# gt1/daccord

Measured on AMD Instinct MI355X. Metric: corrected Mbase/s (whole node), synthetic 20x PacBio piles, higher is better.
Workload: dtype u64+f64; 1 GPU; BASELINE.json configs[1] (10k A-reads x 10 kb x 20x, k=14, one MI355X): synthetic 10000 A-reads x 10000 b x 20x, 15% error (ins 80/del 13.3/sub 6.7), k=14, w=40, a=10, tspace=100; piles_total=10000, piles_rank0=10000, overlaps_rank0=319252, windows_rank0=9969965, trace_blocks_rank0=17906701, corrected_bases_total=90715992

## Files before the change

daccord_amd/csrc/capi.hip:

```cpp
#include <hip/hip_runtime.h>
#include <vector>
#include <string>
#include <cstring>
#include <cstdio>
#include <cstdlib>
#include <new>
#include "../../include/daccord_hip.h"
#include "batch_plan.hpp"
#include "host_tables.hpp"
#include "window_kernels.hpp"
#include "trace_kernel.hpp"
#include "vote_kernel.hpp"
#include "emit_record.hpp"
#include "context.hpp"

using namespace dacc;


struct PrepBatch
{
	DevOvl const * ovl; uint64_t novl; uint8_t const * trace; uint32_t trace_bytes;
	uint32_t * blk_ovl; uint32_t * blk_b0;
};

// ... 297 lines not shown

int dacc_create(dacc_ctx ** out, dacc_params const * p)
{
	if ( !out || !p ) return DACC_EINVAL;
	*out = 0;
	if ( p->klow < 3 || p->khigh > 16 || p->klow > p->khigh || !p->w || !p->a || p->w > DACC_WMAX || p->minfilterfreq < 0 ||
	     p->maxfilterfreq < p->minfilterfreq || p->tspace <= 0 || p->tspace > 512 )
		return DACC_EINVAL;
	if ( readTierSwitches().conflict() ) return DACC_EINVAL;
	int ndev = 0;
	if ( hipGetDeviceCount(&ndev) != hipSuccess || ndev <= 0 || p->device < 0 || p->device >= ndev )
		return DACC_ENODEV;
	if ( hipSetDevice(p->device) != hipSuccess ) return DACC_ENODEV;
	dacc_ctx * c = new (std::nothrow) dacc_ctx;
	if ( !c ) return DACC_ENOMEM;
	c->par = *p; c->device = p->device;
	c->sw = readTierSwitches();
	char const * sc = getenv("DACC_SCHED"); c->env_sched = sc ? atoi(sc) : 1;
	{ char const * td = getenv("DACC_TRACE_DYN"); c->env_trdyn = !(td && td[0] == '0'); }
	char const * ta = getenv("DACC_T7_ADAPT"); c->env_t7adapt = !(ta && ta[0] == '0');
	char const * dr = getenv("DACC_DEBUG_RETRY"); c->env_dbgretry = (dr && dr[0] == '1');
	{ char const * fn = getenv("DACC_FEAS_NEED"); c->env_feasneed = (fn && fn[0] == '0') ? 0u : 1u; }
	{ char const * tf = getenv("DACC_TIE_FAST"); c->env_tiefast = (tf && tf[0] == '0') ? 0u : 1u; }
	if ( hipStreamCreate(&c->stream.h) != hipSuccess ) { delete c; return DACC_EHIP; }
	{ int lo = 0, hi = 0; hipDeviceGetStreamPriorityRange(&lo,&hi); if ( hipStreamCreateWithPriority(&c->stream2.h,hipStreamNonBlocking,hi) != hipSuccess ) { delete c; return DACC_EHIP; } }
	hipEventCreateWithFlags(&c->evFirstTier.h,hipEventDisableTiming); hipEventCreateWithFlags(&c->evEarlyGeneric.h,hipEventDisableTiming); hipEventCreateWithFlags(&c->evPrescan.h,hipEventDisableTiming);
	for ( Event & e : c->ev ) hipEventCreate(&e.h);
	for ( Event & e : c->evEmit ) hipEventCreate(&e.h);
	for ( Event & e : c->evLong ) hipEventCreate(&e.h);
	for ( Event & e : c->evslot ) hipEventCreate(&e.h);
	for ( dacc_ctx::Stage & S : c->st ) hipEventCreate(&S.done.h);
	hipEventCreate(&c->h2dend.h);
	*out = c;
	return DACC_OK;
}

void dacc_destroy(dacc_ctx * c)
{
	if ( !c ) return;
	hipSetDevice(c->device);
	hipStreamSynchronize(c->stream); hipStreamSynchronize(c->stream2);
	delete c;
}

char const * dacc_last_error(dacc_ctx * c) { return c ? c->err.c_str() : "null context"; }

// ... 72 lines not shown
static dacc_ctx::Stage * ranOf(dacc_ctx * c, TierId const id) { return c->st[id].ran ? &c->st[id] : static_cast<dacc_ctx::Stage *>(0); }

struct Pass
{
	WindowBatch WB;
	uint32_t const * list = 0;
	int lastslot = -1;
	bool early = false;
	uint32_t herr[4] = {0,0,0,0};
	size_t symbytes = 0;
};

static WindowBatch windowBatch(dacc_ctx * c)
{
	BatchPlan & BP = c->BP; WindowBatch WB;
	WB.P = c->P; WB.T = c->T; WB.C = BP.caps; WB.bps = c->d_bps.p; WB.boff = c->d_boff.p; WB.rlen = c->d_rlen.p;
	WB.piles = c->d_piles.p; WB.npiles = BP.piles.size(); WB.ovl = c->d_ovl.p; WB.wt_b = c->d_wt_b.p; WB.wt_e = c->d_wt_e.p;
	WB.nwindows = BP.nwindows; WB.wrec = c->d_wrec.p; WB.wout = c->d_wout.p; WB.arena = c->d_arena.p; WB.prof = c->d_prof.p;
	return WB;
}
static FastBatch stageBatch(dacc_ctx * c, WindowBatch const & WB, uint32_t const id, bool const chain = true)
{
	FastBatch FB; FB.W = WB; FB.F = c->BP.stageCaps(id); FB.dpsq_vst = c->d_vst.p; FB.tab32 = c->d_tab32.p; FB.feasneed = c->env_feasneed; FB.tiefast = c->env_tiefast;
	if ( !chain ) return FB;
	FB.hand = c->handcap ? c->d_hand.p : static_cast<uint64_t *>(0); FB.handctr = c->d_handctr.p; FB.handcap = c->handcap; FB.handwords = c->TP.handwords;
#if defined(DACC_LEDGER)
	{ char const * lm = getenv("DACC_LEDGER_MASK"); FB.ledger = lm ? static_cast<uint32_t>(strtoul(lm,0,0)) : 0u; }
#endif
	return FB;
}
static void handsOn(FastBatch & FB, uint32_t * const handon, uint8_t * const slab) { FB.retry = handon; FB.gslab = slab; FB.gstride = FB.F.gbytes; }

static void growHandOver(dacc_ctx * c)
{
	if ( !(c->nruns && c->handwant > c->handcap && !c->nohand) ) return;
	uint64_t cap = c->handwant;
	{ size_t fr = 0, tot = 0; if ( hipMemGetInfo(&fr,&tot) == hipSuccess ) { uint64_t const lim = (static_cast<uint64_t>(fr)/2) / (static_cast<uint64_t>(c->TP.handwords)*8ull); if ( cap > lim ) cap = lim; } else (void)hipGetLastError(); }
	while ( cap && c->d_hand.ensure(static_cast<size_t>(cap)*c->TP.handwords) != hipSuccess ) { (void)hipGetLastError(); cap = cap > 65536 ? cap/2 : 0; }
	c->handcap = static_cast<uint32_t>(cap); c->handwant = cap;
}

static int enqueuePrepAndTrace(dacc_ctx * c)
{
	BatchPlan & BP = c->BP; hipStream_t const s = c->stream;
	HIPCHK(hipMemsetAsync(c->d_err.p,0,4*sizeof(uint32_t),s));
	HIPCHK(hipEventRecord(c->ev[0],s));
// ... 682 lines not shown
```

daccord_amd/csrc/context.hpp:

```cpp
#ifndef DACC_CONTEXT_HPP
#define DACC_CONTEXT_HPP
#include <hip/hip_runtime.h>
#include <cstdlib>
#include <string>
#include <vector>
#include "../../include/daccord_hip.h"
#include "batch_plan.hpp"
#include "host_tables.hpp"
#include "window_main.hpp"
#include "vote_kernel.hpp"

namespace dacc {

template<typename T>
struct DevBuf
{
	T * p = 0; size_t cap = 0;
	DevBuf() = default; DevBuf(DevBuf const &) = delete; DevBuf & operator=(DevBuf const &) = delete;
	~DevBuf() { release(); }
	hipError_t ensure(size_t n)
	{
		if ( n <= cap ) return hipSuccess;
		if ( p ) { hipFree(p); p = 0; cap = 0; }
		hipError_t const e = hipMalloc(reinterpret_cast<void **>(&p),n*sizeof(T));
// ... 53 lines not shown
	std::vector<uint32_t> h_rlen;
	BatchPlan BP;
	DevBuf<DevPile> d_piles; DevBuf<DevOvl> d_ovl; DevBuf<uint32_t> d_ovl_pile; DevBuf<uint8_t> d_trace;
	DevBuf<uint32_t> d_blk_ovl, d_blk_b0, d_wt_b, d_wt_e;
	DevBuf<uint8_t> d_wrec; DevBuf<WindowOut> d_wout; DevBuf<uint8_t> d_arena;
	DevBuf<uint8_t> d_has, d_oc, d_outsym, d_pilebad; DevBuf<uint16_t> d_ld0; DevBuf<uint32_t> d_ocs, d_nfrag, d_err;
	DevBuf<VoteFragment> d_frags; DevBuf<uint64_t> d_fragbase; DevBuf<uint64_t> d_prof;
	DevBuf<uint64_t> d_vst; DevBuf<uint32_t> d_tab32; DevBuf<uint8_t> d_gslab, d_arena2; DevBuf<uint64_t> d_trslab;
	DevBuf<uint32_t> d_retry[TIER_NSLOTS], d_work, d_gearly, d_pregen, d_pregen2, d_pregenlist, d_small;
	DevBuf<uint8_t> d_longslab;
	DevBuf<uint32_t> d_longhand[2];
	DevBuf<uint64_t> d_hand; DevBuf<uint32_t> d_handctr; uint32_t handcap = 0; uint64_t handwant = 0, nruns = 0; bool nohand = false, oom = false;
	bool noslab = false;
	bool tier7_adapt_off = false;
	TierSwitches sw = {}; TierPipeline TP = {};
	struct Stage { bool ran = false; uint32_t grid = 0; DevBuf<uint32_t> handon; DevBuf<uint8_t> slab; Event done; uint32_t const * in = 0;  } st[TIER_NROWS];
	uint32_t nlong[2] = {0,0};
	bool longran[2] = {false,false}; Event evLong[4];
	uint32_t retry_grid = 0, early_grid = 0; int sched = 0;
	uint32_t tr_grid = 0, tr_lds = 0, tr_words = 0, tr_lanes = 0, trace_bytes = 0, win_grid = 0;
	int env_sched = 1, env_dbgretry = 0, env_t7adapt = 1, env_trdyn = 1;
	uint32_t env_feasneed = 1;
	uint32_t env_tiefast = 1;
	std::vector<uint32_t> retry_flags;
	std::vector<dacc_fragment> frags; std::string bases;
	std::vector<int32_t> pile_status; std::vector<std::string> pile_errors; std::string pile_errors_joined;
	std::vector<uint32_t> h_nfrag; std::vector<VoteFragment> h_frags; HostBuf<uint8_t> h_outsym;
	dacc_timing timing = {};
};

}

struct dacc_ctx : dacc::Context {};
#endif
```

daccord_amd/csrc/fast_diag.hpp:

```cpp
#ifndef DACC_FAST_DIAG_HPP
#define DACC_FAST_DIAG_HPP
#if defined(DACC_EMUL)
#include <cstdint>
#include <cstdio>
#include <cstdlib>
#include <vector>
#include <algorithm>
#endif

namespace dacc {

#if defined(DACC_EMUL)
struct FastStats { enum { N = 33 }; uint32_t v[N]; void clear() { for ( int i = 0; i < N; ++i ) v[i] = 0; } void mx(int i, uint32_t x) { if ( x > v[i] ) v[i] = x; } void add(int i, uint32_t x) { v[i] += x; } };
static FastStats g_fstats;
static inline void fstats_dump(int const tier)
{
	static FILE * sf = 0; static bool tried = false;
	if ( !tried ) { tried = true; char const * fn = getenv("DACC_EMUL_STATS"); if ( fn ) sf = fopen(fn,"w"); }
	if ( sf ) { fprintf(sf,"%d",tier); for ( int i = 0; i < FastStats::N; ++i ) fprintf(sf," %u",g_fstats.v[i]); fprintf(sf,"\n"); fflush(sf); }
}
static inline FILE * ftrav_file() { static FILE * f = 0; static bool tried = false; if ( !tried ) { tried = true; char const * fn = getenv("DACC_EMUL_TRAV"); if ( fn ) f = fopen(fn,"w"); } return f; }
#define FSTAT_MX(i,x) g_fstats.mx(i,x)
#define FSTAT_ADD(i,x) g_fstats.add(i,x)
struct FeasIters { std::vector<uint32_t> it, ln; void clear() { it.clear(); ln.clear(); } };
static FeasIters g_feasit;
static inline void feasit_dump()
{
	static FILE * f = 0; static bool tried = false;
	if ( !tried ) { tried = true; char const * fn = getenv("DACC_EMUL_FEAS"); if ( fn ) f = fopen(fn,"w"); }
	if ( !f ) { g_feasit.clear(); return; }
	std::vector<uint32_t> const & it = g_feasit.it; std::vector<uint32_t> const & ln = g_feasit.ln;
	uint64_t tot = 0, lock = 0, locksorted = 0;
	for ( size_t i = 0; i < it.size(); ++i ) tot += it[i];
	for ( size_t i = 0; i < it.size(); i += 64 ) { uint32_t m = 0; for ( size_t q = i; q < it.size() && q < i+64; ++q ) m = std::max(m,it[q]); lock += m; }
	std::vector< std::pair<uint32_t,uint32_t> > P; for ( size_t i = 0; i < it.size(); ++i ) P.push_back(std::make_pair(ln[i],it[i]));
	std::stable_sort(P.begin(),P.end(),[](std::pair<uint32_t,uint32_t> const & a, std::pair<uint32_t,uint32_t> const & b){ return a.first > b.first; });
	for ( size_t i = 0; i < P.size(); i += 64 ) { uint32_t m = 0; for ( size_t q = i; q < P.size() && q < i+64; ++q ) m = std::max(m,P[q].second); locksorted += m; }
	uint64_t lockcls = 0;
	{
		std::vector< std::pair<uint32_t,uint32_t> > Q; for ( size_t i = 0; i < it.size(); ++i ) { uint32_t c = 0; while ( (2u<<c) <= ln[i] ) ++c; Q.push_back(std::make_pair(c,it[i])); }
		std::stable_sort(Q.begin(),Q.end(),[](std::pair<uint32_t,uint32_t> const & a, std::pair<uint32_t,uint32_t> const & b){ return a.first > b.first; });
		for ( size_t i = 0; i < Q.size(); i += 64 ) { uint32_t m = 0; for ( size_t q = i; q < Q.size() && q < i+64; ++q ) m = std::max(m,Q[q].second); lockcls += m; }
	}
	fprintf(f,"%zu %llu %llu %llu %llu\n",it.size(),(unsigned long long)tot,(unsigned long long)lock,(unsigned long long)locksorted,(unsigned long long)lockcls);
// ... 82 lines not shown
static FeasNeedAudit g_feasneed;
#define FEAS_NEED_UNIT(s,rev,lo0,hi0,lo1,hi1) { if ( !feascount ) g_feasneed.unit(s,rev,lo0,hi0,lo1,hi1); }
#define FEAS_NEED_PROBE(s,rev,p) g_feasneed.probe(s,rev,p);
#define FEAS_NEED_LINK(a,b) g_feasneed.link(a,b);
#define FEAS_OVER() { if ( !feascount ) over(128); }
#define FEAS_NEED_PASS() { if ( lane == 0 ) ++g_feasneed.passes; }
#define FEAS_NEED_DUMP() { if ( lane == 0 && !feascount && g_feasneed.on() ) { FeasNeedAudit & A_ = g_feasneed; ++A_.ntrav; A_.recF += nwF; A_.recR += nwR; A_.mids += nmid; A_.hlek += (H <= static_cast<int64_t>(k)); \
	for ( uint32_t c_ = 0; c_ < nF; ++c_ ) A_.insF += (L.fnode()[c_] != 0xFFFF && L.parF()[c_] != SNONE); for ( uint32_t c_ = 0; c_ < nL; ++c_ ) A_.insL += (L.lnode()[c_] != 0xFFFF && L.parL()[c_] != SNONE); A_.dump(); } }
#else
#define FEAS_ITERS(t,len,n)
#define FEAS_DUMP()
#define FEAS_UNITS(W,nu)
#define FEAS_NODE(j,len,pp,nrows,f)
#define FEAS_FAIL(j,len)
#define FEAS_CASES_DUMP()
#define FEAS_NEED_UNIT(s,rev,lo0,hi0,lo1,hi1)
#define FEAS_NEED_PROBE(s,rev,p)
#define FEAS_NEED_LINK(a,b)
#define FEAS_NEED_DUMP()
#define FEAS_NEED_PASS()
#define FEAS_OVER() over(128);
#define FSTAT_MX(i,x)
#define FSTAT_ADD(i,x)
#endif
}
#endif
```

daccord_amd/csrc/fast_tiers.hpp:

```cpp
#ifndef DACC_FAST_TIERS_HPP
#define DACC_FAST_TIERS_HPP
#include <cstdint>
#include "tier_pipeline.hpp"

namespace dacc {

template<int TIER> struct FastTier;
#if !defined(DACC_RCH01)
#define DACC_RCH01 2
#endif
template<> struct FastTier<1> { typedef uint8_t id_t; typedef uint8_t sid_t; enum : uint32_t { smax = 250, gw = 1, wcapg = 1024, rch = DACC_RCH01, fch = 4, fnw = 2, fnc = 40, idmax = 250, rpstcap = 256, lstr = 64, maxs = 32, precap = 1024, ncap = 776, scap = 112, lcap = 960, wcap = 1024, rccap = 144, fcap = 192, siqcap = 56, blcap = 96, seqcap = 32, psiq = 8, consrow = 64, lscrids = 2048, wide = 0, mins = 0, gmem = 0 }; };
template<> struct FastTier<0> { typedef uint8_t id_t; typedef uint8_t sid_t; enum : uint32_t { smax = 250, gw = 1, wcapg = 768, rch = DACC_RCH01, fch = 4, fnw = 2, fnc = 32, idmax = 250, rpstcap = 256, lstr = 64, maxs = 28, precap = 576, ncap = 524, scap = 88, lcap = 640, wcap = 768, rccap = 96, fcap = 128, siqcap = 56, blcap = 96, seqcap = 32, psiq = 8, consrow = 64, lscrids = 2048, wide = 0, mins = 0, gmem = 0 }; };
template<> struct FastTier<7> { typedef uint8_t id_t; typedef uint8_t sid_t; enum : uint32_t { smax = 250, gw = 1, wcapg = 896, rch = DACC_RCH01, fch = 4, fnw = 2, fnc = 32, idmax = 250, rpstcap = 256, lstr = 64, maxs = 28, precap = 704, ncap = 640, scap = 104, lcap = 800, wcap = 896, rccap = 112, fcap = 148, siqcap = 56, blcap = 96, seqcap = 32, psiq = 8, consrow = 64, lscrids = 2048, wide = 0, mins = 0, gmem = 0 }; };
#if !defined(DACC_T2_NCAP)
#define DACC_T2_NCAP 1536
#endif
#if !defined(DACC_T2_LCAP)
#define DACC_T2_LCAP 2032
#endif
template<> struct FastTier<2> { typedef uint8_t id_t; typedef uint8_t sid_t; enum : uint32_t { smax = 250, gw = 1, wcapg = 3072, rch = 4, fch = 4, fnw = 4, fnc = 64, idmax = 250, rpstcap = 256, lstr = 64, maxs = 96, precap = 2048, ncap = DACC_T2_NCAP, scap = 232, lcap = DACC_T2_LCAP, wcap = 3072, rccap = 256, fcap = 192, siqcap = 96, blcap = 96, seqcap = 48, psiq = 10, consrow = 96, lscrids = 2560, wide = 0, mins = 0, gmem = 0 }; };
template<> struct FastTier<6> { typedef uint8_t id_t; typedef uint8_t sid_t; enum : uint32_t { smax = 250, gw = 1, wcapg = 2048, rch = 2, fch = 8, fnw = 3, fnc = 40, idmax = 250, rpstcap = 256, lstr = 128, maxs = 40, precap = 1024, ncap = 1024, scap = 248, lcap = 1280, wcap = 2048, rccap = 256, fcap = 256, siqcap = 96, blcap = 96, seqcap = 48, psiq = 10, consrow = 96, lscrids = 2560, wide = 0, mins = 0, gmem = 0 }; };

template<> struct FastTier<3> { typedef uint16_t id_t; typedef uint16_t sid_t; enum : uint32_t { smax = 1000, gw = 1, wcapg = 8192, rch = 8, fch = 16, fnw = 4, fnc = 72, idmax = 4000, rpstcap = 768, lstr = 128, maxs = 96, precap = 4096, ncap = 2048, scap = 1024, lcap = 4096, wcap = 8192, rccap = 2048, fcap = 512, siqcap = 256, blcap = 128, seqcap = 48, psiq = 10, consrow = 96, lscrids = 2560, wide = 0, mins = 0, gmem = 0 }; };

template<> struct FastTier<4> { typedef uint8_t id_t; typedef uint8_t sid_t; enum : uint32_t { smax = 250, gw = 1, wcapg = 608, rch = 4, fch = 4, fnw = 2, fnc = 40, idmax = 250, rpstcap = 256, lstr = 64, maxs = 96, precap = 2048, ncap = 256, scap = 48, lcap = 256, wcap = 608, rccap = 128, fcap = 96, siqcap = 56, blcap = 96, seqcap = 48, psiq = 10, consrow = 96, lscrids = 2560, wide = 0, mins = 0, gmem = 0 }; };

template<> struct FastTier<5> { typedef uint16_t id_t; typedef uint8_t sid_t; enum : uint32_t { smax = 250, gw = 0, wcapg = 0, rch = 8, fch = 16, fnw = 4, fnc = 72, idmax = 4000, rpstcap = 768, lstr = 128, maxs = 64, precap = 4096, ncap = 1792, scap = 250, lcap = 2048, wcap = 2040, rccap = 512, fcap = 512, siqcap = 256, blcap = 128, seqcap = 48, psiq = 10, consrow = 96, lscrids = 2560, wide = 0, mins = 0, gmem = 0 }; };

template<> struct FastTier<8> { typedef uint16_t id_t; typedef uint8_t sid_t; enum : uint32_t { smax = 250, gw = 1, wcapg = 6144, rch = 4, fch = 8, fnw = 4, fnc = 64, idmax = 4000, rpstcap = 768, lstr = 128, maxs = 40, precap = 3072, ncap = 2304, scap = 248, lcap = 3072, wcap = 6144, rccap = 640, fcap = 512, siqcap = 96, blcap = 128, seqcap = 96, psiq = 10, consrow = 128, lscrids = 2560, wide = 1, mins = 0, gmem = 0 }; };

template<> struct FastTier<9> { typedef uint16_t id_t; typedef uint16_t sid_t; enum : uint32_t { smax = 500, gw = 1, wcapg = 8192, rch = 16, fch = 16, fnw = 4, fnc = 72, idmax = 4000, rpstcap = 768, lstr = 128, maxs = 64, precap = 4096, ncap = 3072, scap = 512, lcap = 4096, wcap = 8192, rccap = 2048, fcap = 1024, siqcap = 256, blcap = 128, seqcap = 96, psiq = 10, consrow = 128, lscrids = 2560, wide = 1, mins = 0, gmem = 0 }; };

template<> struct FastTier<10> { typedef uint16_t id_t; typedef uint8_t sid_t; enum : uint32_t { smax = 250, gw = 1, wcapg = 6144, rch = 4, fch = 8, fnw = 4, fnc = 64, idmax = 4000, rpstcap = 768, lstr = 128, maxs = 64, precap = 2560, ncap = 2048, scap = 248, lcap = 3072, wcap = 6144, rccap = 896, fcap = 512, siqcap = 128, blcap = 128, seqcap = 48, psiq = 10, consrow = 96, lscrids = 2560, wide = 0, mins = 0, gmem = 0 }; };

template<> struct FastTier<11> { typedef uint16_t id_t; typedef uint8_t sid_t; enum : uint32_t { smax = 250, gw = 1, wcapg = 4096, rch = 4, fch = 8, fnw = 4, fnc = 72, idmax = 4000, rpstcap = 768, lstr = 128, maxs = 96, precap = 4096, ncap = 1536, scap = 248, lcap = 2048, wcap = 4096, rccap = 640, fcap = 384, siqcap = 128, blcap = 128, seqcap = 48, psiq = 10, consrow = 96, lscrids = 2560, wide = 0, mins = 0, gmem = 0 }; };

template<> struct FastTier<12> { typedef uint16_t id_t; typedef uint16_t sid_t; enum : uint32_t { smax = 1000, gw = 1, wcapg = 8192, rch = 8, fch = 16, fnw = 4, fnc = 72, idmax = 4000, rpstcap = 768, lstr = 128, maxs = 250, precap = 8192, ncap = 2048, scap = 1024, lcap = 4096, wcap = 8192, rccap = 2048, fcap = 512, siqcap = 256, blcap = 128, seqcap = 48, psiq = 10, consrow = 96, lscrids = 2560, wide = 0, mins = 96, gmem = 0 }; };

template<> struct FastTier<13> { typedef uint16_t id_t; typedef uint16_t sid_t; enum : uint32_t { smax = 2000, gw = 1, wcapg = 16384, rch = 16, fch = 16, fnw = 4, fnc = 72, idmax = 4000, rpstcap = 768, lstr = 128, maxs = 250, precap = 16384, ncap = 4096, scap = 2048, lcap = 8192, wcap = 16384, rccap = 4096, fcap = 1024, siqcap = 512, blcap = 128, seqcap = 48, psiq = 10, consrow = 96, lscrids = 4096, wide = 0, mins = 0, gmem = 1 }; };
template<> struct FastTier<14> { typedef uint16_t id_t; typedef uint16_t sid_t; enum : uint32_t { smax = 1000, gw = 1, wcapg = 16384, rch = 16, fch = 16, fnw = 4, fnc = 72, idmax = 4000, rpstcap = 768, lstr = 128, maxs = 250, precap = 16384, ncap = 6144, scap = 1024, lcap = 8192, wcap = 16384, rccap = 4096, fcap = 2048, siqcap = 512, blcap = 128, seqcap = 96, psiq = 10, consrow = 128, lscrids = 4096, wide = 1, mins = 0, gmem = 1 }; };
template<> struct FastTier<15> { typedef uint16_t id_t; typedef uint16_t sid_t; enum : uint32_t { smax = 2000, gw = 1, wcapg = 32768, rch = 16, fch = 16, fnw = 4, fnc = 72, idmax = 4000, rpstcap = 768, lstr = 128, maxs = 1000, precap = 16384, ncap = 4096, scap = 2048, lcap = 8192, wcap = 32768, rccap = 4096, fcap = 1024, siqcap = 512, blcap = 128, seqcap = 48, psiq = 10, consrow = 96, lscrids = 4096, wide = 0, mins = 250, gmem = 1 }; };

static_assert(uint32_t(FastTier<15>::mins) == VDEEP_MINS && uint32_t(FastTier<13>::maxs) == VDEEP_MINS,"the very deep stage takes what the last stage refuses at its string count");
template<> struct FastTier<16> { typedef uint16_t id_t; typedef uint16_t sid_t; enum : uint32_t { smax = 4000, gw = 1, wcapg = 65536, rch = 16, fch = 16, fnw = 4, fnc = 72, idmax = 8000, rpstcap = 768, lstr = 128, maxs = 2000, precap = 16384, ncap = 8190, scap = 4096, lcap = 16384, wcap = 65536, rccap = 4096, fcap = 1024, siqcap = 512, blcap = 128, seqcap = 48, psiq = 10, consrow = 96, lscrids = 4096, wide = 0, mins = 250, gmem = 1 }; };
static_assert(uint32_t(FastTier<16>::mins) == VDEEP_MINS && uint32_t(FastTier<15>::maxs) == XDEEP_MINS,"the deepest stage takes what the very deep stage hands on with more than 250 strings");
template<> struct FastTier<18> { typedef uint16_t id_t; typedef uint16_t sid_t; enum : uint32_t { smax = 12000, gw = 1, wcapg = 131072, rch = 16, fch = 16, fnw = 4, fnc = 72, idmax = 24000, rpstcap = 768, lstr = 128, maxs = 5001, precap = 16384, ncap = 16384, scap = 12288, lcap = 49152, wcap = 131072, rccap = 4096, fcap = 1024, siqcap = 512, blcap = 128, seqcap = 48, psiq = 10, consrow = 96, lscrids = 4096, wide = 0, mins = 250, gmem = 1 }; };
static_assert(uint32_t(FastTier<18>::mins) == VDEEP_MINS && uint32_t(FastTier<16>::maxs) == FDEEP_MINS,"the full-depth stage takes what the deepest stage hands on with more than 250 strings");
template<> struct FastTier<19> { typedef uint16_t id_t; typedef uint16_t sid_t; enum : uint32_t { smax = 4000, gw = 1, wcapg = 98304, rch = 64, fch = 16, fnw = 4, fnc = 72, idmax = 8000, rpstcap = 768, lstr = 128, maxs = 1000, precap = 16384, ncap = 8190, scap = 4096, lcap = 16384, wcap = 98304, rccap = 16384, fcap = 2048, siqcap = 512, blcap = 128, seqcap = 96, psiq = 10, consrow = 128, lscrids = 16384, wide = 1, mins = 250, gmem = 1 }; };
static_assert(uint32_t(FastTier<19>::mins) == VDEEP_MINS && uint32_t(FastTier<14>::maxs) == VDEEP_MINS && uint32_t(FastTier<19>::maxs) == FastTier<15>::maxs,"the wide deep stage takes what the last stage of a wide batch refuses at its string count");
template<> struct FastTier<17> { typedef uint16_t id_t; typedef uint16_t sid_t; enum : uint32_t { smax = 1000, gw = 1, wcapg = 16384, rch = 16, fch = 16, fnw = 8, fnc = 72, idmax = 4000, rpstcap = 768, lstr = 256, maxs = 250, precap = 16384, ncap = 6144, scap = 1024, lcap = 8192, wcap = 16384, rccap = 4096, fcap = 4096, siqcap = 512, blcap = 128, seqcap = 96, psiq = 10, consrow = 128, lscrids = 4096, wide = 1, mins = 0, gmem = 1, oneslab = 1 }; };
template<typename CT, typename = void> struct FastOneSlab { enum : uint32_t { value = 0 }; };
template<typename CT> struct FastOneSlab<CT,decltype(void(CT::oneslab))> { enum : uint32_t { value = (CT::oneslab != 0) ? 1u : 0u }; };

}
#endif
```

daccord_amd/csrc/fast_window.hpp:

```cpp
#ifndef DACC_FAST_WINDOW_HPP
#define DACC_FAST_WINDOW_HPP
#include "wave.hpp"
#include "dev_types.hpp"
#include "arena.hpp"
#include "window_main.hpp"
#include "tier_pipeline.hpp"
#include "fast_tiers.hpp"
#include "fast_layout.hpp"
#include "fast_diag.hpp"
#include "emit_record.hpp"

namespace dacc {

enum { WS_RETRY = 4 };
enum { FNOPAR = 0xFF };
enum { FSEQCAP = 48 };

struct FastBatch
{
	WindowBatch W;
	FastCaps F = {};
	uint64_t const * dpsq_vst = 0;
	uint32_t * retry = 0;
	uint32_t * gearly = 0;
// ... 31 lines not shown
struct FastEngine
{
	typedef typename CT::id_t id_t;
	typedef typename CT::sid_t sid_t;
	enum : uint32_t { SB = 8u*sizeof(sid_t), SMASK = (1u<<SB)-1u, SNONE = SMASK, SMAX = CT::smax };
	FastLds<CT> L; DevTables T; DevParams P;
	uint32_t nrows, nsup;
	uint64_t const * vst;
	enum : bool { GW = (CT::gw != 0) };
	uint8_t * gslab;
	uint32_t const * gtab;
	struct G4 { uint32_t x, y, z, w; };
	int lane; uint32_t flags;
#if defined(DACC_LEDGER)
	uint32_t ledger;
#endif
	uint64_t * prof;
	uint32_t mao, k; uint64_t kmask;
	uint32_t npre, nlast, nn, nmfirst, nmlast;
	uint32_t n0, npool, nlinks, nwF, nwR;
	uint32_t nF, nL;
	uint32_t feasneed;
	uint32_t tiefast;

#if defined(DACC_EMUL)
	bool feascount, feasapplied; uint32_t nwFall, nwRall;
	DEV bool feasNeedOn() const { char const * e = getenv("DACC_FEAS_NEED"); return !(e && e[0] == '0'); }
	DEV bool tieFastOn() const { char const * e = getenv("DACC_TIE_FAST"); return !(e && e[0] == '0'); }
#else
	static constexpr bool feascount = false;
	DEV bool feasNeedOn() const { return feasneed != 0; }
	DEV bool tieFastOn() const { return tiefast != 0; }
#endif
#if defined(DACC_EMUL)
	DEV void over_(uint32_t b, int line) { flags |= b; static char const * ov = getenv("DACC_EMUL_OVER"); if ( ov ) fprintf(stderr,"[over] tier maxs=%d line %d bits 0x%x nn=%u n0=%u npool=%u nF=%u nL=%u nwF=%u nwR=%u rstop=%u\n",int(CT::maxs)*10000+int(CT::ncap),line,b,nn,n0,npool,nF,nL,nwF,nwR,rstop); }
	#define over(b) over_(b,__LINE__)
#else
	DEV void over(uint32_t b) { flags |= b; }
#endif
#if defined(DACC_PROFILE) && !defined(DACC_EMUL)
	DEV void pcount(int id, uint64_t v) { if ( prof ) atomicAdd(reinterpret_cast<unsigned long long *>(prof+id),static_cast<unsigned long long>(v)); }
	DEV uint64_t pclock() { return clock64(); }
#else
	DEV void pcount(int, uint64_t) {}
	DEV uint64_t pclock() { return 0; }
#endif

#if defined(DACC_PROFILE) && !defined(DACC_EMUL)
	#define SITE_T0 uint64_t _ps = clock64();
	#define SITE_RESET { _ps = clock64(); }
	#define SITE(id) { uint64_t const _n = clock64(); if ( prof && lane == static_cast<int>(__builtin_ctzll(__builtin_amdgcn_ballot_w64(true))) ) { atomicAdd(reinterpret_cast<unsigned long long *>(prof+32+(id)),static_cast<unsigned long long>(_n-_ps)); atomicAdd(reinterpret_cast<unsigned long long *>(prof+80+(id)),1ull); } _ps = clock64(); }
	#define PROFX_T0 uint64_t _px = clock64();
	#define PROFX(id) { uint64_t const _n = clock64(); if ( lane == 0 && prof ) atomicAdd(reinterpret_cast<unsigned long long *>(prof+(id)),static_cast<unsigned long long>(_n-_px)); _px = _n; }
#else
	#define PROFX_T0
// ... 1896 lines not shown
		if ( conslen > CONSROW ) { over(4096); return ~0u; }
		uint32_t qf = path, qr = rp;
		uint32_t const ns = nf > nr ? nf : nr;
		for ( uint32_t t = 0; t < ns; ++t )
		{
			if ( t < nf ) { dst[nf-1-t] = L.f_stretch()[qf]; qf = L.f_parent()[qf]; }
			if ( t < nr ) { dst[nf+t] = L.rc_stretch()[qr]; qr = L.rc_parent()[qr]; }
		}
		return nf+nr;
	}
	DEV uint32_t decodeSeq(LDSQ sid_t const * seq, uint32_t const n, LDSQ uint8_t * dst) const
	{
		uint32_t o = 0;
		uint32_t const firstv = L.nv()[L.sfirst()[seq[0]]];
		for ( uint32_t i = 0; i < k; ++i ) dst[o++] = (firstv >> (2*(k-1-i))) & 3;
		for ( uint32_t ii = 0; ii < n; ++ii )
		{
			uint32_t const s = seq[ii]; LDSQ uint16_t const * Lk = L.links() + L.slink()[s];
			uint32_t const len = L.sslen()[s];
			for ( uint32_t j = 1; j < len; ++j ) dst[o++] = L.nv()[Lk[j]] & 3;
		}
		return o;
	}
	DEV bool scoreInterval(uint32_t const sbase, uint32_t const nacc2, uint32_t const front, int64_t const candlen, int64_t const lmin, int64_t const lmax,
		uint32_t & sub, uint32_t & sup, uint32_t & mi) const
	{
		uint32_t lo = 0, hi = nacc2;
		while ( lo < hi ) { uint32_t const mid = (lo+hi)>>1; if ( L.rc_front()[sbase+mid] < front ) lo = mid+1; else hi = mid; }
		uint32_t e = lo;
		while ( e < nacc2 && L.rc_front()[sbase+e] == front ) ++e;
		if ( e == lo ) return false;
		int64_t bllo = lmin + static_cast<int64_t>(k) - candlen; if ( bllo < 0 ) bllo = 0;
		int64_t blhi = lmax + static_cast<int64_t>(k) - candlen; if ( blhi < 0 ) blhi = 0;
		uint32_t const bllo16 = static_cast<uint16_t>(bllo), blhi16 = static_cast<uint16_t>(blhi);
		sub = lo;
		while ( sub < e && L.rc_sbl()[sbase+sub] < bllo16 ) ++sub;
		sup = sub;
		while ( sup < e && !(blhi16 < L.rc_sbl()[sbase+sup]) ) ++sup;
		if ( sub == sup ) return false;
		mi = sub; uint32_t mr = L.rc_arw()[sbase+sub];
		for ( uint32_t i = sub+1; i < sup; ++i ) { uint32_t const r = L.rc_arw()[sbase+i]; if ( r > mr ) { mi = i; mr = r; } }
		return true;
	}
	DEV bool scoreNext(uint32_t const sbase, uint32_t const left, uint32_t const right, uint32_t const current, uint32_t & bi) const
	{
		uint32_t const v = L.rc_arw()[sbase+current];
// ... 995 lines not shown
				if ( tie && !tiefast ) exact = true;
				wv_sync();
			}
			if ( exact )
			{
#if defined(DACC_LEDGER)
				FCC keep_[WSZ >= 16 ? 1 : 16]; for ( uint32_t c = lane; c < nkept; c += WSZ ) keep_[c/WSZ] = ldget(L.cdh()+c);
#endif
				LEDGER_REP(18)
				{
#if defined(DACC_LEDGER)
				wv_sync(); for ( uint32_t c = lane; c < nkept; c += WSZ ) ldput(L.cdh()+c,keep_[c/WSZ]); wv_sync();
#endif
				if ( lane == 0 )
				{
					uint32_t nh = nkept, nch = 0, na = 0;
					while ( nh ) { FCC const c = ldget(L.cdh()); spop<FCC,true>(L.cdh(),nh); spush<FCC,false>(L.ch(),nch,c); }
					while ( nch ) { ldput(L.acc()+na,ldget(L.ch())); ++na; spop<FCC,false>(L.ch(),nch); }
				}
				}
				if ( lane == 0 ) FSTAT_ADD(32,tiefast ? 1u : 0u);
				wv_sync();
			}
			for ( uint32_t c = lane; c < nkept; c += WSZ )
			{
				uint32_t const slot = L.acc()[c].o, n = L.acc()[c].l & 0xFF;
				uint32_t len = 0;
				LEDGER_REP(19) len = decodeSeq(L.cseq()+FSEQCAP*slot,n,L.consL()+c*CONSROW);
				L.acc()[c].o = c*CONSROW; L.acc()[c].l = len;
			}
			wv_sync();
			LEDGER_REP(14)
			for ( uint32_t t = lane; t < nkept*mao; t += WSZ )
			{
				uint32_t const c = t / mao, j = t - c*mao;
				L.canderr()[t] = myersDistance(j,L.consL() + L.acc()[c].o,L.acc()[c].l);
			}
			wv_sync();
			for ( uint32_t c = lane; c < nkept; c += WSZ )
			{
				uint32_t s = 0;
				for ( uint32_t j = 0; j < mao; ++j ) s += L.canderr()[c*mao+j];
				L.accerr()[c] = s;
			}
			wv_sync();
			{
				LDSQ uint32_t * const serr = reinterpret_cast<LDSQ uint32_t *>(L.canderr());
				static_assert(16*CT::maxs >= 64 && (FastLds<CT>::o_canderr & 3) == 0,"sorted error sums borrow the candidate error bytes");
				for ( uint32_t c = lane; c < nkept; c += WSZ )
				{
					uint32_t const e = L.accerr()[c];
					uint32_t rank = 0;
// ... 244 lines not shown

template<typename CT>
DEV int processWindowFast(FastBatch const & FB, uint64_t const widx, LDSQ uint8_t * lds, bool const resume = false)
{
	WindowBatch const & B = FB.W;
	FastEngine<CT> E;
#if defined(DACC_EMUL)
	{ char const * pz = getenv("DACC_EMUL_POISON"); if ( pz ) __builtin_memset(static_cast<void *>(&E),atoi(pz),sizeof(E)); }
#endif
	if ( B.pregen && ((B.pregen[widx>>5] >> (widx&31)) & 1) ) return FW_DONE;
	E.mao = 0; E.k = 0; E.kmask = 0; E.npre = E.nlast = E.nn = E.nmfirst = E.nmlast = 0; E.n0 = E.npool = E.nlinks = E.nwF = E.nwR = 0; E.nF = E.nL = 0;
	E.nsiq = E.ncdh = E.nacc = 0; E.rstop = 0; E.roundT0 = 0; E.cfree = 0; E.pvpath = E.pvrp = E.pvnf = 0; E.pvcl = 0; E.nmid = 0; E.midbase = 0; E.nLmagic = 0;
	E.T = B.T; E.P = B.P; E.nrows = FB.F.nrows; E.nsup = FB.F.nsup; E.vst = FB.dpsq_vst;
	E.gslab = 0; E.gtab = FB.tab32; E.sfresh = true; E.sdirty = false;
	if ( CT::gw )
	{
#if defined(DACC_EMUL)
		E.gslab = FB.gslab;
#else
		E.gslab = FB.gslab + static_cast<uint64_t>(blockIdx.x)*FB.gstride;
#endif
		if constexpr ( FastOneSlab<CT>::value != 0 ) E.gslab = (uint8_t *)(lds) + FastLds<CT>::g_base;
	}
	E.lane = wv_lane(); E.flags = 0; E.prof = B.prof; E.feasneed = FB.feasneed; E.tiefast = FB.tiefast;
#if defined(DACC_EMUL)
	E.feascount = false; E.feasapplied = false; E.nwFall = E.nwRall = 0;
#endif
#if defined(DACC_LEDGER)
	E.ledger = FB.ledger;
#endif
#if defined(DACC_PROFILE) && !defined(DACC_EMUL)
	uint64_t * const prof = E.prof;
#endif
#if defined(DACC_EMUL)
	g_fstats.clear();
#endif
	E.L.base = lds;
	FastLds<CT> const & L = E.L;
	int const lane = E.lane;
	PROF_T0
	int32_t curff = B.P.maxff;
	uint32_t hslot = 0;
	bool const handable = FB.hand != 0 && B.P.klow == B.P.khigh && CT::gw != 0;
	if ( resume && B.P.klow == B.P.khigh )
	{
		WindowOut const prev = B.wout[widx];
		if ( prev.status == WS_RETRY && prev.filterfreq <= B.P.maxff && prev.filterfreq >= B.P.minff )
// ... 240 lines not shown
```

daccord_amd/csrc/window_main.hpp:

```cpp
#ifndef DACC_WINDOW_MAIN_HPP
#define DACC_WINDOW_MAIN_HPP
#include "dbg_window.hpp"

namespace dacc {

struct WindowBatch
{
	DevParams P = {};
	DevTables T = {};
	ArenaCaps C = {};
	uint8_t const * bps = 0; uint64_t const * boff = 0; uint32_t const * rlen = 0;
	DevPile const * piles = 0; uint32_t npiles = 0;
	DevOvl const * ovl = 0;
	uint32_t const * wt_b = 0; uint32_t const * wt_e = 0;
	uint64_t nwindows = 0;
	uint8_t * wrec = 0;
	WindowOut * wout = 0;
	uint8_t * arena = 0;
	uint64_t * prof = 0;
	uint32_t const * pregen = 0;
};

DEV uint8_t readBase(uint8_t const * bps, uint64_t const off, uint32_t const len, bool const inv, uint32_t const p)
{
	uint32_t const q = inv ? (len-1-p) : p;
	uint8_t const b = (bps[off+(q>>2)] >> (6-2*(q&3))) & 3;
	return inv ? (3-b) : b;
}

DEV void windowInterval(uint32_t const l, uint32_t const a, uint32_t const w, uint32_t const y, uint32_t & s, uint32_t & e)
{
	if ( static_cast<uint64_t>(y)*a + w <= l ) { s = y*a; e = s+w; }
	else { s = l-w; e = l; }
}

// ... 179 lines not shown
```

Measured before the change: 42.66 Mbase/s.

## Decode kept consensus candidates as per-stretch lane tasks instead of per-candidate lanes

Adds a task-parallel decode of kept consensus candidates for the small tiers (0, 1, 6, 7). Each stretch of a candidate becomes one lane task, with wave prefix scans placing the output offsets, so the wavefront no longer sits mostly idle when there are few candidates. It reuses the CH and accerr LDS regions as scratch and falls back to the old per-candidate decode when there are too many tasks or a candidate is empty. An env switch, DACC_DECODE_TASKS, turns it off, and an emulation-only diagnostic dump is added.

After: 42.91 Mbase/s (median of 6 runs). No clear change (+0.6%).

```diff
diff --git a/daccord_amd/csrc/capi.hip b/daccord_amd/csrc/capi.hip
--- a/daccord_amd/csrc/capi.hip
+++ b/daccord_amd/csrc/capi.hip
@@ -343,6 +343,7 @@
 	char const * dr = getenv("DACC_DEBUG_RETRY"); c->env_dbgretry = (dr && dr[0] == '1');
 	{ char const * fn = getenv("DACC_FEAS_NEED"); c->env_feasneed = (fn && fn[0] == '0') ? 0u : 1u; }
 	{ char const * tf = getenv("DACC_TIE_FAST"); c->env_tiefast = (tf && tf[0] == '0') ? 0u : 1u; }
+	{ char const * dt = getenv("DACC_DECODE_TASKS"); c->env_dectasks = (dt && dt[0] == '0') ? 0u : 1u; }
 	if ( hipStreamCreate(&c->stream.h) != hipSuccess ) { delete c; return DACC_EHIP; }
 	{ int lo = 0, hi = 0; hipDeviceGetStreamPriorityRange(&lo,&hi); if ( hipStreamCreateWithPriority(&c->stream2.h,hipStreamNonBlocking,hi) != hipSuccess ) { delete c; return DACC_EHIP; } }
 	hipEventCreateWithFlags(&c->evFirstTier.h,hipEventDisableTiming); hipEventCreateWithFlags(&c->evEarlyGeneric.h,hipEventDisableTiming); hipEventCreateWithFlags(&c->evPrescan.h,hipEventDisableTiming);
@@ -461,6 +462,7 @@
 static FastBatch stageBatch(dacc_ctx * c, WindowBatch const & WB, uint32_t const id, bool const chain = true)
 {
 	FastBatch FB; FB.W = WB; FB.F = c->BP.stageCaps(id); FB.dpsq_vst = c->d_vst.p; FB.tab32 = c->d_tab32.p; FB.feasneed = c->env_feasneed; FB.tiefast = c->env_tiefast;
+	FB.W.decodelanes = c->env_dectasks ? 0u : 1u;
 	if ( !chain ) return FB;
 	FB.hand = c->handcap ? c->d_hand.p : static_cast<uint64_t *>(0); FB.handctr = c->d_handctr.p; FB.handcap = c->handcap; FB.handwords = c->TP.handwords;
 #if defined(DACC_LEDGER)
diff --git a/daccord_amd/csrc/context.hpp b/daccord_amd/csrc/context.hpp
--- a/daccord_amd/csrc/context.hpp
+++ b/daccord_amd/csrc/context.hpp
@@ -99,6 +99,7 @@
 	int env_sched = 1, env_dbgretry = 0, env_t7adapt = 1, env_trdyn = 1;
 	uint32_t env_feasneed = 1;
 	uint32_t env_tiefast = 1;
+	uint32_t env_dectasks = 1;
 	std::vector<uint32_t> retry_flags;
 	std::vector<dacc_fragment> frags; std::string bases;
 	std::vector<int32_t> pile_status; std::vector<std::string> pile_errors; std::string pile_errors_joined;
diff --git a/daccord_amd/csrc/fast_diag.hpp b/daccord_amd/csrc/fast_diag.hpp
--- a/daccord_amd/csrc/fast_diag.hpp
+++ b/daccord_amd/csrc/fast_diag.hpp
@@ -20,6 +20,13 @@
 	if ( sf ) { fprintf(sf,"%d",tier); for ( int i = 0; i < FastStats::N; ++i ) fprintf(sf," %u",g_fstats.v[i]); fprintf(sf,"\n"); fflush(sf); }
 }
 static inline FILE * ftrav_file() { static FILE * f = 0; static bool tried = false; if ( !tried ) { tried = true; char const * fn = getenv("DACC_EMUL_TRAV"); if ( fn ) f = fopen(fn,"w"); } return f; }
+static inline FILE * fdecode_file() { static FILE * f = 0; static bool tried = false; if ( !tried ) { tried = true; char const * fn = getenv("DACC_EMUL_DECODE"); if ( fn ) f = fopen(fn,"w"); } return f; }
+#define DECODE_CASES(nkept,exact,tasks) { FILE * const f_ = lane == 0 ? fdecode_file() : 0; if ( f_ ) { \
+	uint32_t nt_ = 0, single_ = 0, len1_ = 0, m8_ = 0, n8_ = 0, none_ = 0; \
+	for ( uint32_t c_ = 0; c_ < (nkept); ++c_ ) { uint32_t const slot_ = L.acc()[c_].o, n_ = L.acc()[c_].l & 0xFF; uint32_t len_ = k; nt_ += n_; single_ += (n_ == 1); none_ += (n_ == 0); \
+		for ( uint32_t i_ = 0; i_ < n_; ++i_ ) { uint32_t const sl_ = L.sslen()[L.cseq()[FSEQCAP*slot_+i_]]; len1_ += (sl_ == 1); len_ += sl_ ? sl_-1 : 0u; } \
+		if ( len_ & 7u ) ++n8_; else ++m8_; } \
+	fprintf(f_,"%d %u %u %u %u %u %u %u %d %d\n",int(CT::maxs)*10000+int(CT::ncap),uint32_t(nkept),nt_,single_,len1_,m8_,n8_,none_,(exact) ? 1 : 0,(tasks) ? 1 : 0); fflush(f_); } }
 #define FSTAT_MX(i,x) g_fstats.mx(i,x)
 #define FSTAT_ADD(i,x) g_fstats.add(i,x)
 struct FeasIters { std::vector<uint32_t> it, ln; void clear() { it.clear(); ln.clear(); } };
@@ -148,6 +155,7 @@
 #define FEAS_OVER() over(128);
 #define FSTAT_MX(i,x)
 #define FSTAT_ADD(i,x)
+#define DECODE_CASES(nkept,exact,tasks)
 #endif
 }
 #endif
diff --git a/daccord_amd/csrc/fast_tiers.hpp b/daccord_amd/csrc/fast_tiers.hpp
--- a/daccord_amd/csrc/fast_tiers.hpp
+++ b/daccord_amd/csrc/fast_tiers.hpp
@@ -9,9 +9,9 @@
 #if !defined(DACC_RCH01)
 #define DACC_RCH01 2
 #endif
-template<> struct FastTier<1> { typedef uint8_t id_t; typedef uint8_t sid_t; enum : uint32_t { smax = 250, gw = 1, wcapg = 1024, rch = DACC_RCH01, fch = 4, fnw = 2, fnc = 40, idmax = 250, rpstcap = 256, lstr = 64, maxs = 32, precap = 1024, ncap = 776, scap = 112, lcap = 960, wcap = 1024, rccap = 144, fcap = 192, siqcap = 56, blcap = 96, seqcap = 32, psiq = 8, consrow = 64, lscrids = 2048, wide = 0, mins = 0, gmem = 0 }; };
-template<> struct FastTier<0> { typedef uint8_t id_t; typedef uint8_t sid_t; enum : uint32_t { smax = 250, gw = 1, wcapg = 768, rch = DACC_RCH01, fch = 4, fnw = 2, fnc = 32, idmax = 250, rpstcap = 256, lstr = 64, maxs = 28, precap = 576, ncap = 524, scap = 88, lcap = 640, wcap = 768, rccap = 96, fcap = 128, siqcap = 56, blcap = 96, seqcap = 32, psiq = 8, consrow = 64, lscrids = 2048, wide = 0, mins = 0, gmem = 0 }; };
-template<> struct FastTier<7> { typedef uint8_t id_t; typedef uint8_t sid_t; enum : uint32_t { smax = 250, gw = 1, wcapg = 896, rch = DACC_RCH01, fch = 4, fnw = 2, fnc = 32, idmax = 250, rpstcap = 256, lstr = 64, maxs = 28, precap = 704, ncap = 640, scap = 104, lcap = 800, wcap = 896, rccap = 112, fcap = 148, siqcap = 56, blcap = 96, seqcap = 32, psiq = 8, consrow = 64, lscrids = 2048, wide = 0, mins = 0, gmem = 0 }; };
+template<> struct FastTier<1> { typedef uint8_t id_t; typedef uint8_t sid_t; enum : uint32_t { smax = 250, gw = 1, wcapg = 1024, rch = DACC_RCH01, fch = 4, fnw = 2, fnc = 40, idmax = 250, rpstcap = 256, lstr = 64, maxs = 32, precap = 1024, ncap = 776, scap = 112, lcap = 960, wcap = 1024, rccap = 144, fcap = 192, siqcap = 56, blcap = 96, seqcap = 32, psiq = 8, consrow = 64, lscrids = 2048, wide = 0, mins = 0, gmem = 0, dectasks = 1 }; };
+template<> struct FastTier<0> { typedef uint8_t id_t; typedef uint8_t sid_t; enum : uint32_t { smax = 250, gw = 1, wcapg = 768, rch = DACC_RCH01, fch = 4, fnw = 2, fnc = 32, idmax = 250, rpstcap = 256, lstr = 64, maxs = 28, precap = 576, ncap = 524, scap = 88, lcap = 640, wcap = 768, rccap = 96, fcap = 128, siqcap = 56, blcap = 96, seqcap = 32, psiq = 8, consrow = 64, lscrids = 2048, wide = 0, mins = 0, gmem = 0, dectasks = 1 }; };
+template<> struct FastTier<7> { typedef uint8_t id_t; typedef uint8_t sid_t; enum : uint32_t { smax = 250, gw = 1, wcapg = 896, rch = DACC_RCH01, fch = 4, fnw = 2, fnc = 32, idmax = 250, rpstcap = 256, lstr = 64, maxs = 28, precap = 704, ncap = 640, scap = 104, lcap = 800, wcap = 896, rccap = 112, fcap = 148, siqcap = 56, blcap = 96, seqcap = 32, psiq = 8, consrow = 64, lscrids = 2048, wide = 0, mins = 0, gmem = 0, dectasks = 1 }; };
 #if !defined(DACC_T2_NCAP)
 #define DACC_T2_NCAP 1536
 #endif
@@ -19,7 +19,7 @@
 #define DACC_T2_LCAP 2032
 #endif
 template<> struct FastTier<2> { typedef uint8_t id_t; typedef uint8_t sid_t; enum : uint32_t { smax = 250, gw = 1, wcapg = 3072, rch = 4, fch = 4, fnw = 4, fnc = 64, idmax = 250, rpstcap = 256, lstr = 64, maxs = 96, precap = 2048, ncap = DACC_T2_NCAP, scap = 232, lcap = DACC_T2_LCAP, wcap = 3072, rccap = 256, fcap = 192, siqcap = 96, blcap = 96, seqcap = 48, psiq = 10, consrow = 96, lscrids = 2560, wide = 0, mins = 0, gmem = 0 }; };
-template<> struct FastTier<6> { typedef uint8_t id_t; typedef uint8_t sid_t; enum : uint32_t { smax = 250, gw = 1, wcapg = 2048, rch = 2, fch = 8, fnw = 3, fnc = 40, idmax = 250, rpstcap = 256, lstr = 128, maxs = 40, precap = 1024, ncap = 1024, scap = 248, lcap = 1280, wcap = 2048, rccap = 256, fcap = 256, siqcap = 96, blcap = 96, seqcap = 48, psiq = 10, consrow = 96, lscrids = 2560, wide = 0, mins = 0, gmem = 0 }; };
+template<> struct FastTier<6> { typedef uint8_t id_t; typedef uint8_t sid_t; enum : uint32_t { smax = 250, gw = 1, wcapg = 2048, rch = 2, fch = 8, fnw = 3, fnc = 40, idmax = 250, rpstcap = 256, lstr = 128, maxs = 40, precap = 1024, ncap = 1024, scap = 248, lcap = 1280, wcap = 2048, rccap = 256, fcap = 256, siqcap = 96, blcap = 96, seqcap = 48, psiq = 10, consrow = 96, lscrids = 2560, wide = 0, mins = 0, gmem = 0, dectasks = 1 }; };
 
 template<> struct FastTier<3> { typedef uint16_t id_t; typedef uint16_t sid_t; enum : uint32_t { smax = 1000, gw = 1, wcapg = 8192, rch = 8, fch = 16, fnw = 4, fnc = 72, idmax = 4000, rpstcap = 768, lstr = 128, maxs = 96, precap = 4096, ncap = 2048, scap = 1024, lcap = 4096, wcap = 8192, rccap = 2048, fcap = 512, siqcap = 256, blcap = 128, seqcap = 48, psiq = 10, consrow = 96, lscrids = 2560, wide = 0, mins = 0, gmem = 0 }; };
 
@@ -51,6 +51,8 @@
 template<> struct FastTier<17> { typedef uint16_t id_t; typedef uint16_t sid_t; enum : uint32_t { smax = 1000, gw = 1, wcapg = 16384, rch = 16, fch = 16, fnw = 8, fnc = 72, idmax = 4000, rpstcap = 768, lstr = 256, maxs = 250, precap = 16384, ncap = 6144, scap = 1024, lcap = 8192, wcap = 16384, rccap = 4096, fcap = 4096, siqcap = 512, blcap = 128, seqcap = 96, psiq = 10, consrow = 128, lscrids = 4096, wide = 1, mins = 0, gmem = 1, oneslab = 1 }; };
 template<typename CT, typename = void> struct FastOneSlab { enum : uint32_t { value = 0 }; };
 template<typename CT> struct FastOneSlab<CT,decltype(void(CT::oneslab))> { enum : uint32_t { value = (CT::oneslab != 0) ? 1u : 0u }; };
+template<typename CT, typename = void> struct FastDecodeTasks { enum : uint32_t { value = 0 }; };
+template<typename CT> struct FastDecodeTasks<CT,decltype(void(CT::dectasks))> { enum : uint32_t { value = (CT::dectasks != 0) ? 1u : 0u }; };
 
 }
 #endif
diff --git a/daccord_amd/csrc/fast_window.hpp b/daccord_amd/csrc/fast_window.hpp
--- a/daccord_amd/csrc/fast_window.hpp
+++ b/daccord_amd/csrc/fast_window.hpp
@@ -77,15 +77,19 @@
 	uint32_t nF, nL;
 	uint32_t feasneed;
 	uint32_t tiefast;
+	uint32_t decodelanes;
+	enum : bool { DECTASKS = (FastDecodeTasks<CT>::value != 0) };
 
 #if defined(DACC_EMUL)
 	bool feascount, feasapplied; uint32_t nwFall, nwRall;
 	DEV bool feasNeedOn() const { char const * e = getenv("DACC_FEAS_NEED"); return !(e && e[0] == '0'); }
 	DEV bool tieFastOn() const { char const * e = getenv("DACC_TIE_FAST"); return !(e && e[0] == '0'); }
+	DEV bool decodeTasksOn() const { char const * e = getenv("DACC_DECODE_TASKS"); return !(e && e[0] == '0'); }
 #else
 	static constexpr bool feascount = false;
 	DEV bool feasNeedOn() const { return feasneed != 0; }
 	DEV bool tieFastOn() const { return tiefast != 0; }
+	DEV bool decodeTasksOn() const { return decodelanes == 0; }
 #endif
 #if defined(DACC_EMUL)
 	DEV void over_(uint32_t b, int line) { flags |= b; static char const * ov = getenv("DACC_EMUL_OVER"); if ( ov ) fprintf(stderr,"[over] tier maxs=%d line %d bits 0x%x nn=%u n0=%u npool=%u nF=%u nL=%u nwF=%u nwR=%u rstop=%u\n",int(CT::maxs)*10000+int(CT::ncap),line,b,nn,n0,npool,nF,nL,nwF,nwR,rstop); }
@@ -2028,6 +2032,69 @@
 		}
 		return o;
 	}
+	enum : uint32_t { DT_CLEN = 16, DT_CAP = (FastLds<CT>::e_canderr - FastLds<CT>::o_accerr)/2 };
+	DEV bool decodeKeptTasks(uint32_t const nkept) const
+	{
+		static_assert(FSEQCAP <= 64 && sizeof(FCC)*16 >= 2*(DT_CLEN+16) && FastLds<CT>::e_accerr == FastLds<CT>::o_canderr && FastLds<CT>::o_accerr > FastLds<CT>::o_acc,
+			"task decode: 6 bit stretch index, 5 bit slot; scratch in CH and in the error sums and candidate errors, which follow ACC");
+		LDSQ uint16_t * const pfx = reinterpret_cast<LDSQ uint16_t *>(L.ch());
+		LDSQ uint16_t * const clen = pfx + DT_CLEN;
+		LDSQ uint16_t * const tab = reinterpret_cast<LDSQ uint16_t *>(L.accerr());
+		uint32_t ntask = 0, none = 0;
+		for ( uint32_t c0 = 0; c0 < nkept; c0 += WSZ )
+		{
+			uint32_t const c = c0 + lane;
+			uint32_t const n = c < nkept ? (L.acc()[c].l & 0xFF) : 0u;
+			uint32_t tot; uint32_t const pre = ntask + wv_scan_excl(n,tot); ntask += tot;
+			if ( c < nkept )
+			{
+				none |= n ? 0u : 1u;
+				uint32_t const e = c | (L.acc()[c].o << 10);
+				if ( pre + n <= DT_CAP ) for ( uint32_t ii = 0; ii < n; ++ii ) tab[pre+ii] = static_cast<uint16_t>(e | (ii << 4) | (ii+1 == n ? 0x8000u : 0u));
+			}
+		}
+		if ( wv_any(none) || ntask > DT_CAP ) return false;
+		wv_sync();
+		uint32_t done = 0;
+		for ( uint32_t t0 = 0; t0 < ntask; t0 += WSZ )
+		{
+			bool const on = t0 + lane < ntask;
+			uint32_t e = 0, slen = 1, lk = 0, firstv = 0;
+			if ( on )
+			{
+				e = tab[t0+lane];
+				uint32_t const s = L.cseq()[FSEQCAP*((e >> 10) & 31u) + ((e >> 4) & 63u)];
+				slen = L.sslen()[s]; lk = L.slink()[s];
+				if ( !(e & 0x3F0u) ) firstv = L.nv()[L.sfirst()[s]];
+			}
+			uint32_t const c = e & 15u;
+			bool const head = on && !(e & 0x3F0u);
+			uint32_t const nb = (on && slen) ? slen-1 : 0u;
+			uint32_t tot; uint32_t const pre = done + wv_scan_excl(nb,tot); done += tot;
+			if ( head ) pfx[c] = static_cast<uint16_t>(pre);
+			wv_sync();
+			if ( on )
+			{
+				LDSQ uint8_t * const dst = L.consL() + c*CONSROW;
+				uint32_t o = k + pre - pfx[c];
+				if ( e & 0x8000u ) clen[c] = static_cast<uint16_t>(o + nb);
+				if ( head ) for ( uint32_t i = 0; i < k; ++i ) dst[i] = (firstv >> (2*(k-1-i))) & 3;
+				LDSQ uint16_t const * const Lk = L.links() + lk;
+				for ( uint32_t j = 1; j < slen; j += 4, o += 4 )
+				{
+					uint32_t const r = slen - j, j1 = r > 1 ? j+1 : j, j2 = r > 2 ? j+2 : j1, j3 = r > 3 ? j+3 : j2;
+					uint32_t const a0 = Lk[j], a1 = Lk[j1], a2 = Lk[j2], a3 = Lk[j3];
+					uint32_t const v0 = L.nv()[a0], v1 = L.nv()[a1], v2 = L.nv()[a2], v3 = L.nv()[a3];
+					dst[o] = v0 & 3;
+					if ( r > 1 ) dst[o+1] = v1 & 3;
+					if ( r > 2 ) dst[o+2] = v2 & 3;
+					if ( r > 3 ) dst[o+3] = v3 & 3;
+				}
+			}
+		}
+		wv_sync();
+		return true;
+	}
 	DEV bool scoreInterval(uint32_t const sbase, uint32_t const nacc2, uint32_t const front, int64_t const candlen, int64_t const lmin, int64_t const lmax,
 		uint32_t & sub, uint32_t & sup, uint32_t & mi) const
 	{
@@ -3069,12 +3136,31 @@
 				if ( lane == 0 ) FSTAT_ADD(32,tiefast ? 1u : 0u);
 				wv_sync();
 			}
+			if constexpr ( DECTASKS )
+			{
+				bool dtasks = decodeTasksOn();
+				DECODE_CASES(nkept,exact,dtasks)
+				if ( dtasks ) { LEDGER_REP(19) dtasks = decodeKeptTasks(nkept); }
+				if ( dtasks )
+					for ( uint32_t c = lane; c < nkept; c += WSZ ) { L.acc()[c].o = c*CONSROW; L.acc()[c].l = reinterpret_cast<LDSQ uint16_t const *>(L.ch())[DT_CLEN+c]; }
+				else
+					for ( uint32_t c = lane; c < nkept; c += WSZ )
+					{
+						uint32_t const slot = L.acc()[c].o, n = L.acc()[c].l & 0xFF;
+						uint32_t len = 0;
+						LEDGER_REP(19) len = decodeSeq(L.cseq()+FSEQCAP*slot,n,L.consL()+c*CONSROW);
+						L.acc()[c].o = c*CONSROW; L.acc()[c].l = len;
+					}
+			}
+			else
+			{
 			for ( uint32_t c = lane; c < nkept; c += WSZ )
 			{
 				uint32_t const slot = L.acc()[c].o, n = L.acc()[c].l & 0xFF;
 				uint32_t len = 0;
 				LEDGER_REP(19) len = decodeSeq(L.cseq()+FSEQCAP*slot,n,L.consL()+c*CONSROW);
 				L.acc()[c].o = c*CONSROW; L.acc()[c].l = len;
+			}
 			}
 			wv_sync();
 			LEDGER_REP(14)
@@ -3365,7 +3451,7 @@
 #endif
 		if constexpr ( FastOneSlab<CT>::value != 0 ) E.gslab = (uint8_t *)(lds) + FastLds<CT>::g_base;
 	}
-	E.lane = wv_lane(); E.flags = 0; E.prof = B.prof; E.feasneed = FB.feasneed; E.tiefast = FB.tiefast;
+	E.lane = wv_lane(); E.flags = 0; E.prof = B.prof; E.feasneed = FB.feasneed; E.tiefast = FB.tiefast; E.decodelanes = B.decodelanes;
 #if defined(DACC_EMUL)
 	E.feascount = false; E.feasapplied = false; E.nwFall = E.nwRall = 0;
 #endif
diff --git a/daccord_amd/csrc/window_main.hpp b/daccord_amd/csrc/window_main.hpp
--- a/daccord_amd/csrc/window_main.hpp
+++ b/daccord_amd/csrc/window_main.hpp
@@ -11,6 +11,7 @@
 	ArenaCaps C = {};
 	uint8_t const * bps = 0; uint64_t const * boff = 0; uint32_t const * rlen = 0;
 	DevPile const * piles = 0; uint32_t npiles = 0;
+	uint32_t decodelanes = 0;
 	DevOvl const * ovl = 0;
 	uint32_t const * wt_b = 0; uint32_t const * wt_e = 0;
 	uint64_t nwindows = 0;
```
